# LANL-Bioinformatics/PCRamp

Measured on AMD Instinct MI355X. Metric: primer-pair x target amplification evals/sec, higher is better.
Workload: dtype u32

## Files before the change

### pcramp_amd/csrc/pcr_device.hip

```cpp
#include <hip/hip_runtime.h>
#include <cstring>
#include <rocprim/device/device_radix_sort.hpp>

#include <stdint.h>
#include <string.h>
#include <math.h>
#include <stdlib.h>
#include <string>
#include <vector>
#include <chrono>
#include <algorithm>
#include <unordered_map>
#include <type_traits>
#include <thread>
#include <mutex>
#include <condition_variable>
#include <functional>
#include <memory>

#include "../../include/pcramp_hip.h"
#include "pcr_host.hpp"

using pcrhost::Planes;

// ... 528 lines not shown
	uint32_t bucket_cap = 64;
	DevBuf<uint32_t> irr_perm; uint32_t irr_size_count[256];
	DevBuf<uint4> planes;
	DevBuf<uint32_t> valid, nib, tb, blk_seq, tile_seq, tile_pos0, irr_off, degen_tiles;
	uint32_t *valid_d() const { return valid.p + S2_VALID_FRONT; }
	uint32_t *tb_d() const { return tb.p + S2_TB_FRONT; }
	DevBuf<uint8_t> tile_degen; uint32_t n_degen_tiles = 0;
	DevBuf<TileDesc> tile_desc;
	DevBuf<uint64_t> d_len, d_blk_off, d_nblk_real;
	DevBuf<uint8_t> d_active;
	std::vector<uint8_t> has_eos; DevBuf<uint8_t> d_has_eos;
	DevBuf<IrrDev> irr;
	DevBuf<IrrScan> irr_scan;
	DevBuf<uint32_t> irx_first, irx_last, irx_words, irx_sums; bool irx_valid = false, irx_usable = false;
	uint32_t irr_n_multi = 0;
	DevBuf<uint32_t> pix_first, pix_last, pix_sums, blk_info, blk_local, blk_tile0; DevBuf<uint4> pix_ent; std::vector<uint32_t> pix_count_h; uint64_t pix_generation = 0; bool pix_valid = false, pix_usable = false;
	DevBuf<uint8_t> codes; DevBuf<uint64_t> d_code_off; bool have_codes = false;
	bool have_db = false;
	uint32_t n_entries = 0;
	uint32_t db_cap = 0;
	uint64_t n_slots = 0;
	DevBuf<DevEntry> db;
	DevBuf<uint32_t> touched;
	DevBuf<uint32_t> ctrl;
	uint32_t n_touched = 0;
	bool touched_built = false;
	uint32_t *d_seg_hi = nullptr;
	void release()
	{
		d_weight.release(); tile_desc.release(); irr_scan.release(); irx_first.release(); irx_last.release(); irx_words.release(); irx_sums.release(); pix_first.release(); pix_last.release(); pix_ent.release(); pix_sums.release(); blk_info.release(); blk_local.release(); blk_tile0.release(); irr_perm.release(); planes.release(); valid.release(); nib.release(); tb.release(); degen_tiles.release(); tile_degen.release(); blk_seq.release(); tile_seq.release(); tile_pos0.release();
		irr_off.release(); d_len.release(); d_blk_off.release();
		d_nblk_real.release(); d_active.release(); d_has_eos.release(); irr.release(); db.release(); touched.release(); ctrl.release(); codes.release(); d_code_off.release();
	}
};

}

struct HostPool {
	std::vector<std::thread> th;
	std::mutex m; std::condition_variable cv_go, cv_done;
	std::function<void(unsigned)> fn; unsigned n_parts = 0, next = 0, pending = 0; uint64_t gen = 0; bool stop = false;
	explicit HostPool(unsigned n_workers){ for(unsigned i = 0;i < n_workers;++i) th.emplace_back([this]{ work(); }); }
	~HostPool(){ { std::lock_guard<std::mutex> lk(m); stop = true; } cv_go.notify_all(); for(std::thread &t : th) t.join(); }
	unsigned size() const { return (unsigned)th.size(); }
	void work()
// ... 35 lines not shown
	pcrhost::PackFilter filt;
	SeqSet sets[PCR_N_SETS];
	DevBuf<uint32_t> best, counters, mask, status;
	int scan_version = 3;
	bool force_seed1 = false;
	std::vector<uint32_t> s2_seeds; std::vector<uint4> s2_masks; std::vector<uint8_t> s2_floors;
	std::vector<uint32_t> s2_group_end, s2_group_offmask, s2_group_or, s2_group_nor;
	struct S2Key { uint32_t a, c, g, t, floor_; bool operator==(const S2Key &o) const { return a == o.a && c == o.c && g == o.g && t == o.t && floor_ == o.floor_; } };
	struct S2KeyHash { size_t operator()(const S2Key &k) const { uint64_t h = 0x9E3779B97F4A7C15ull; for(uint32_t v : {k.a, k.c, k.g, k.t, k.floor_}){ h ^= v; h *= 0x100000001B3ull; h ^= h >> 29; } return (size_t)h; } };
	struct S2Entry { std::vector<uint32_t> seeds;  uint32_t off_mask; bool seedable; uint4 mask;
		std::vector<uint32_t> chunks; uint32_t chunks_total = 0; uint64_t chunks_gen = 0;  };
	std::unordered_map<S2Key, S2Entry, S2KeyHash> s2_cache;
	std::vector<pcrhost::Seed> s2_tmp;
	struct S3Launch { Seed3Slices W; uint32_t n_chunks, per_wg, slice_cap, n_irr_wg; };
	std::vector<S3Launch> s3_launch;
	std::vector<uint32_t> s3_prefix; bool no_seed3 = false, s3_attr_set = false;
	bool s2_attr_set = false; uint32_t s2_dbg = 0; bool no_irr_index = false;
	std::vector<uint32_t> s1_seeds; std::unordered_map<S2Key, S2Entry, S2KeyHash> s1_cache;
	DevBuf<uint32_t> s1_image, s1_heads, s1_multi, s1_part;
	bool host_seed_tables = false;
	DevBuf<Hit> hits;
	DevBuf<uint64_t> bits_fr, bits_rf;
	DevBuf<OligoDev> oligos;
	DevBuf<SwJob> sw_jobs; DevBuf<SwOut> sw_out; DevBuf<uint8_t> sw_q, sw_qlen, sw_t, entry_codes, entry_lens;
	DevBuf<AmpRec> amp_recs, amp_recs2; DevBuf<BgPairDev> bg_pairs;
	DevBuf<uint64_t> amp_keys; DevBuf<uint32_t> amp_pkeys, amp_pair_start; DevBuf<uint8_t> sort_tmp;
	DevBuf<thermo::Job> th_jobs; DevBuf<thermo::JobOut> th_out; DevBuf<int> th_dg; DevBuf<uint2> th_map; DevBuf<uint32_t> th_bad;
	float th_dg_salt = -1.0f;
	DevBuf<unsigned long long> th_dbg; bool th_attr_set = false;
	std::vector<thermo::Job> th_host_jobs; std::vector<thermo::JobOut> th_host_res;
	uint8_t *sw_pin = nullptr, *sw_pin_dev = nullptr; hipEvent_t sw_done[2] = {nullptr, nullptr};
// ... 193 lines not shown
	hipLaunchKernelGGL(k_scan_blocks, dim3(n_blocks), dim3(1024), 0, ctx->stream, S.irx_last.p, S.irx_first.p, IRX_KEYS, S.irx_sums.p);
	hipLaunchKernelGGL(k_scan_sums, dim3(1), dim3(1024), 0, ctx->stream, S.irx_sums.p, n_blocks);
	hipLaunchKernelGGL(k_scan_add, dim3(n_blocks), dim3(1024), 0, ctx->stream, S.irx_first.p, S.irx_last.p, IRX_KEYS, S.irx_sums.p);
	HIP_TRY(hipGetLastError());
	if(S.n_irr){
		hipLaunchKernelGGL(k_irx_scatter, dim3((S.n_irr + 255)/256), dim3(256), 0, ctx->stream, S.irr.p, S.n_irr, S.irx_last.p, S.irx_words.p);
		HIP_TRY(hipGetLastError());
	}
	S.irx_valid = true;
	return PCR_OK;
}

int ensure_pos_index(pcr_ctx *ctx, SeqSet &S)
{
	if(S.pix_valid) return PCR_OK;
	S.pix_valid = true; S.pix_usable = false;
	if(S.total_blocks == 0 || S.total_blocks*32 >= (uint64_t(1) << 32) - 64) return PCR_OK;
	int rc;
	if((rc = S.pix_first.ensure(PIX_CODES + 4)) != PCR_OK) return rc;
	if((rc = S.pix_last.ensure(PIX_CODES + 4)) != PCR_OK) return rc;
	const uint32_t n_blocks = (PIX_CODES + 4095u)/4096u;
	if((rc = S.pix_sums.ensure(n_blocks + 4)) != PCR_OK) return rc;
	if((rc = S.pix_ent.ensure(S.total_blocks*32 + 64)) != PCR_OK) return rc;
	{
		if(S.n >= (1u << 30)){ return PCR_OK; }
		if((rc = S.blk_info.ensure(S.total_blocks + 1)) != PCR_OK) return rc;
		if((rc = S.blk_local.ensure(S.total_blocks + 1)) != PCR_OK) return rc;
		std::vector<uint32_t> tile0((size_t)S.n + 1);
		uint64_t t0 = 0;
		for(uint32_t q = 0;q < S.n;++q){ tile0[q] = (uint32_t)t0; t0 += (S.len[q] >= 32) ? (S.len[q] - 7 + TILE_POS - 1)/TILE_POS : 0; }
		tile0[S.n] = (uint32_t)t0;
		if(t0 >= (uint64_t(1) << 32)) return PCR_OK;
		if((rc = S.blk_tile0.ensure((size_t)S.n + 1)) != PCR_OK) return rc;
		HIP_TRY(hipMemcpyAsync(S.blk_tile0.p, tile0.data(), ((size_t)S.n + 1)*sizeof(uint32_t), hipMemcpyHostToDevice, ctx->stream));
		hipLaunchKernelGGL(k_blk_info, dim3((unsigned)((S.total_blocks + 255)/256)), dim3(256), 0, ctx->stream, S.blk_seq.p, S.d_blk_off.p, S.d_len.p,
			S.blk_tile0.p, S.tile_degen.p, S.d_active.p, S.total_blocks, S.blk_info.p, S.blk_local.p);
		HIP_TRY(hipGetLastError());
		HIP_TRY(hipStreamSynchronize(ctx->stream));
	}
	HIP_TRY(hipMemsetAsync(S.pix_last.p, 0, (size_t)PIX_CODES*sizeof(uint32_t), ctx->stream));
	const unsigned grid = (unsigned)((S.total_blocks + 255)/256);
	hipLaunchKernelGGL(k_pix_build<false>, dim3(grid), dim3(256), 0, ctx->stream, S.tb_d(), S.blk_seq.p, S.d_blk_off.p, S.d_len.p, S.total_blocks, S.pix_last.p, (uint4 *)nullptr);
	hipLaunchKernelGGL(k_scan_blocks, dim3(n_blocks), dim3(1024), 0, ctx->stream, S.pix_last.p, S.pix_first.p, PIX_CODES, S.pix_sums.p);
	hipLaunchKernelGGL(k_scan_sums, dim3(1), dim3(1024), 0, ctx->stream, S.pix_sums.p, n_blocks);
	hipLaunchKernelGGL(k_scan_add, dim3(n_blocks), dim3(1024), 0, ctx->stream, S.pix_first.p, S.pix_last.p, PIX_CODES, S.pix_sums.p);
	hipLaunchKernelGGL(k_pix_build<true>, dim3(grid), dim3(256), 0, ctx->stream, S.tb_d(), S.blk_seq.p, S.d_blk_off.p, S.d_len.p, S.total_blocks, S.pix_last.p, S.pix_ent.p);
	HIP_TRY(hipGetLastError());
	{
		std::vector<uint32_t> first(PIX_CODES), last(PIX_CODES);
		HIP_TRY(hipMemcpyAsync(first.data(), S.pix_first.p, (size_t)PIX_CODES*sizeof(uint32_t), hipMemcpyDeviceToHost, ctx->stream));
		HIP_TRY(hipMemcpyAsync(last.data(), S.pix_last.p, (size_t)PIX_CODES*sizeof(uint32_t), hipMemcpyDeviceToHost, ctx->stream));
		HIP_TRY(hipStreamSynchronize(ctx->stream));
		S.pix_count_h.resize(PIX_CODES);
		for(uint32_t c = 0;c < PIX_CODES;++c) S.pix_count_h[c] = last[c] - first[c];
		static uint64_t generations = 0;
		S.pix_generation = ++generations;
	}
	S.pix_usable = true;
	return PCR_OK;
}

int run_valid(pcr_ctx *ctx, SeqSet &S, uint64_t first_block, uint64_t n_blocks)
{
	if(n_blocks == 0) return PCR_OK;
	const unsigned threads = 256;
	const unsigned grid = (unsigned)((n_blocks + threads - 1)/threads);
	hipLaunchKernelGGL(k_valid, dim3(grid), dim3(threads), 0, ctx->stream, S.planes.p, S.d_blk_off.p, S.blk_seq.p,
		S.d_nblk_real.p, S.valid_d(), S.total_blocks, ctx->filt.max_degen, ctx->filt.gc_ok, first_block, n_blocks);
	HIP_TRY(hipGetLastError());
	return PCR_OK;
}

int build_tile_desc(pcr_ctx *ctx, SeqSet &S)
// ... 822 lines not shown
		const uint32_t *P = ctx->s3_prefix.data() + g_prefix;
		g_prefix += (size_t)ns + 1;
		pcr_ctx::S3Launch &L = ctx->s3_launch[g];
		L.n_irr_wg = with_irr ? std::min<uint32_t>((ns + 16u*(uint32_t)(wg_threads/64) - 1u)/(16u*(uint32_t)(wg_threads/64)), G_all/4u) : 0u;
		const uint32_t G = G_all - L.n_irr_wg;
		L.n_chunks = P[ns]; L.per_wg = std::max<uint32_t>(1u, (L.n_chunks + G - 1u)/G); L.slice_cap = 2;
		if(ns == 0) continue;
		uint32_t at = 0;
		for(uint32_t w = 0;w <= G;++w){
			const uint64_t target = (uint64_t)w*L.per_wg;
			while(at + 1u < ns && P[at + 1u] <= target) ++at;
			L.W.start[w] = at;
		}
		for(uint32_t w = G + 1;w <= S3_MAX_WG;++w) L.W.start[w] = at;
		for(uint32_t w = 0;w < G;++w) L.slice_cap = std::max(L.slice_cap, std::min(L.W.start[w + 1] + 2u, ns + 1u) - L.W.start[w]);
		if(17*(size_t)ctx->s2_group_nor[g] + 8*(size_t)L.slice_cap + 64 > S3_LDS_BUDGET) return false;
	}
	return true;
}

void plan_seed1(pcr_ctx *ctx, const std::vector<pcrhost::Candidate> &cand, std::vector<uint32_t> &or_seed, std::vector<uint32_t> &or_plain, uint32_t &irr_off_mask)
{
	const uint32_t n_or = 2*(uint32_t)cand.size();
	std::vector<uint32_t> &out = ctx->s1_seeds;
	out.clear();
	irr_off_mask = 0;
	if(ctx->s1_cache.size() > 16384) ctx->s1_cache.clear();
	std::vector<const pcr_ctx::S2Entry *> ent(n_or);
	size_t total = 0;
	for(uint32_t o = 0;o < n_or;++o){
		const pcrhost::Candidate &c = cand[o >> 1];
// ... 239 lines not shown
		&& ctx->s3_prefix.size() == ctx->s2_seeds.size() + ctx->s2_group_end.size();
	bool dev_tables = false;
	if(!use_seed2 && ctx->scan_version == 3 && !ctx->host_seed_tables && !optimize_5 && !optimize_3 && n_or <= S1_MAX_OR){
		plan_seed1(ctx, cand, or_seed, or_plain, irr_off_mask);
		dev_tables = true;
	}
	if(use_seed2 || dev_tables){  }
	else if(ctx->scan_version == 3 && n_or <= 65535){
		const int prc = plan_seed_host(ctx, cand, H, or_seed, or_plain, irr_off_mask);
		if(ctx->seed_count.size() == 65536){ for(const pcrhost::Seed &sd : H.seeds){ ctx->seed_count[sd.code] = 0; ctx->seed_own[sd.code] = 0; } }
		if(prc != PCR_OK) return prc;
	}
	else{ for(uint32_t o = 0;o < n_or;++o) or_plain.push_back(o); }
	SeedTables ST; memset(&ST, 0, sizeof(ST));
	Seed2Tables ST2; memset(&ST2, 0, sizeof(ST2));
	const uint32_t *d_s3_prefix = nullptr;
	const size_t n_seeds = use_seed2 ? ctx->s2_seeds.size() : dev_tables ? ctx->s1_seeds.size() : H.seeds.size() + H.n_inherited;
	if(ctx->debug_log) fprintf(stderr, "[pcramp] scan plan: %u candidates, %zu seeded orientations (%zu seeds), %zu plain, %u/%u IUPAC tiles, %u-slot buckets\n",
		ncand, or_seed.size(), n_seeds, or_plain.size(), S.n_degen_tiles, S.n_tiles, S.bucket_cap);
	Scan2Tables tab_plain, tab_seedset;
	const bool need_plain = (ctx->scan_version != 1) && !or_plain.empty();
	const bool need_seedset = !or_seed.empty() && S.n_degen_tiles > 0;
	if(need_plain) build_scan2_tables(cand, or_plain, tab_plain);
	if(need_seedset) build_scan2_tables(cand, or_seed, tab_seedset);
	const uint32_t *d_tab_plain = nullptr, *d_bias_plain = nullptr, *d_map_plain = nullptr;
	const uint32_t *d_tab_seedset = nullptr, *d_bias_seedset = nullptr, *d_map_seedset = nullptr;
	{
		size_t bytes = ncand*(2*sizeof(uint4) + sizeof(uint32_t)) + 1024;
		bytes += (tab_plain.tab.size() + tab_plain.bias.size() + or_plain.size() + 256)*sizeof(uint32_t);
		bytes += (tab_seedset.tab.size() + tab_seedset.bias.size() + or_seed.size() + 256)*sizeof(uint32_t);
		bytes += (H.image.size() + H.heads.size() + H.multi.size() + 64)*sizeof(uint32_t);
		std::vector<uint4> &masks2 = ctx->s2_masks; std::vector<uint8_t> &floors2 = ctx->s2_floors;
		if(use_seed2){
			floors2.assign(((size_t)n_or + 15) & ~size_t(15), 0);
			for(uint32_t o = 0;o < n_or;++o) floors2[o] = (uint8_t)std::min<uint32_t>(cand[o >> 1].floor_, 255u);
			bytes += masks2.size()*sizeof(uint4) + floors2.size() + ctx->s2_seeds.size()*sizeof(uint32_t) + 512;
			if(use_seed3) bytes += ctx->s3_prefix.size()*sizeof(uint32_t) + 64;
		}
		const bool build_tables = dev_tables && !or_seed.empty();
		if(build_tables) bytes += ctx->s1_seeds.size()*sizeof(uint32_t) + 256;
		std::vector<OligoDev> ol;
		size_t bits_bytes = 0;
		bool fuse = false;
		if(fa && fa->n_pairs){
			bits_bytes = (size_t)fa->n_pairs*((S.n + 63)/64)*sizeof(uint64_t);
			fuse = ((uintptr_t)fa->d_fr % 16 == 0) && ((uintptr_t)fa->d_rf % 16 == 0) && (bits_bytes % 16 == 0);
			if(fuse){ build_oligos(fa->pairs, fa->n_pairs, fa->a, ol); bytes += ol.size()*sizeof(OligoDev) + 64; }
		}
		timer.next(1);
		{
			const uint64_t gen = S.ctrl.generation;
			if((rc = S.ctrl.ensure(8 + 2*(size_t)S.n + 4)) != PCR_OK) return rc;
// ... 26 lines not shown
			ST.multi = H.multi.empty() ? ST.heads : st.put(H.multi.data(), H.multi.size());
		}
		const uint32_t *d_s1_seeds = nullptr;
		if(build_tables){
			d_s1_seeds = st.put(ctx->s1_seeds.data(), ctx->s1_seeds.size());
			if((rc = ctx->s1_image.ensure(SEED_IMAGE_WORDS)) != PCR_OK) return rc;
			if((rc = ctx->s1_heads.ensure(2*(size_t)S1_MAX_SEEDS)) != PCR_OK) return rc;
			if((rc = ctx->s1_multi.ensure(S1_MAX_SEEDS)) != PCR_OK) return rc;
			ST.image = ctx->s1_image.p; ST.heads = ctx->s1_heads.p; ST.multi = ctx->s1_multi.p; ST.flat = 1;
		}
		if(use_seed2){
			ST2.seeds = st.put(ctx->s2_seeds.data(), ctx->s2_seeds.size());
			ST2.masks = st.put(masks2.data(), masks2.size());
			ST2.floors = st.put(floors2.data(), floors2.size());
			ST2.n_seeds = (uint32_t)ctx->s2_seeds.size(); ST2.n_or = n_or;
			if(use_seed3) d_s3_prefix = st.put(ctx->s3_prefix.data(), ctx->s3_prefix.size());
		}
		if(fuse){
			fa->d_oligos = st.put(ol.data(), ol.size());
			fa->staged = true;
			if(lean) st.seal(ctx->mail_seq + 1);
			else if((rc = st.ship(S.ctrl.p, (8 + 2*(size_t)S.n)*sizeof(uint32_t), fa->d_fr, bits_bytes, fa->d_rf, bits_bytes, ctx->mail_seq + 1)) != PCR_OK) return rc;
		}
		else if((rc = st.ship(S.ctrl.p, (8 + 2*(size_t)S.n)*sizeof(uint32_t), nullptr, 0, nullptr, 0, ctx->mail_seq + 1)) != PCR_OK) return rc;
		if(build_tables){
			if((rc = ctx->s1_part.ensure(2*S1_GROUPS)) != PCR_OK) return rc;
			hipLaunchKernelGGL(k_seed_tables<false>, dim3(S1_GROUPS), dim3(S1_BUILD_THREADS), 0, ctx->stream, d_s1_seeds, (uint32_t)ctx->s1_seeds.size(),
				ctx->s1_part.p, ctx->s1_image.p, ctx->s1_heads.p, ctx->s1_multi.p);
			hipLaunchKernelGGL(k_seed_tables<true>, dim3(S1_GROUPS), dim3(S1_BUILD_THREADS), 0, ctx->stream, d_s1_seeds, (uint32_t)ctx->s1_seeds.size(),
				ctx->s1_part.p, ctx->s1_image.p, ctx->s1_heads.p, ctx->s1_multi.p);
			HIP_TRY(hipGetLastError());
// ... 57 lines not shown
						Tg.masks = ST2.masks + (size_t)or0; Tg.floors = ST2.floors + or0; Tg.n_or = g_or; Tg.or_base = or0;
						g_begin = ctx->s2_group_end[g];
						if(Tg.n_seeds == 0){ g_prefix += 1u; continue; }
						const size_t dyn = (size_t)g_or*sizeof(uint4) + (((size_t)g_or + 15) & ~size_t(15)) + 8*((size_t)Tg.n_seeds + 64) + 16;
						IrrArgs2 IA; IA.scan = S.irr_scan.p; IA.irr = S.irr.p; IA.n_live = n_live;
						IA.off_mask = ctx->s2_group_offmask[g];
						IA.exhaustive = first_launch ? 1u : 0u;
						IA.ix_first = IA.ix_last = IA.ix_words = nullptr; IA.min_cws = std::min<uint32_t>(min_oligo_length, 255u);
						if(!or_plain.empty()){
							IA.off_mask = 0;
							if(!first_launch) IA.n_live = 0;
						}
						else if(irr_by_index){
							IA.ix_first = S.irx_first.p; IA.ix_last = S.irx_last.p; IA.ix_words = S.irx_words.p; IA.n_live = 0;
						}
						if(ctx->debug_log) fprintf(stderr, "[pcramp] k_seed2: %u workgroups, %u seeds of orientations %u..%u (group %zu of %zu), %zu + %zu B of LDS\n", sgrid.x, Tg.n_seeds,
							or0, or0 + g_or - 1, g + 1, ctx->s2_group_end.size(), sizeof(S2Shared), dyn);
						S2Clear Z = { nullptr, 0u, nullptr, 0u, nullptr };
						if(lean && !cleared_bits){
							Z.z0 = (uint4 *)fa->d_fr; Z.z1 = (uint4 *)fa->d_rf; Z.n0 = Z.n1 = (uint32_t)(lean_bits_bytes/16); Z.ctrl = d_counters;
							cleared_bits = true;
						}
						if(use_seed3){
							Seed3Tables T3; T3.seeds = Tg.seeds; T3.chunk_prefix = d_s3_prefix + g_prefix; T3.masks = Tg.masks; T3.floors = Tg.floors;
							g_prefix += Tg.n_seeds + 1u;
							T3.n_seeds = Tg.n_seeds; T3.n_or = Tg.n_or; T3.or_base = Tg.or_base;
							T3.pix_first = S.pix_first.p; T3.pix_last = S.pix_last.p; T3.pix_ent = S.pix_ent.p;
							Seed3Set Q3 = { S.valid_d(), S.blk_info.p, S.blk_local.p, S.d_active.p };
							int s3_wg = 0;
							const uint32_t G = seed3_grid(ctx, &s3_wg);
							const pcr_ctx::S3Launch &L3 = ctx->s3_launch[g];
							T3.n_chunks = L3.n_chunks; T3.per_wg = L3.per_wg; T3.slice_cap = L3.slice_cap;
							T3.n_irr_wg = IA.ix_first ? L3.n_irr_wg : 0u;
							const Seed3Slices &W3 = L3.W;
							const size_t dyn3 = (size_t)g_or*sizeof(uint4) + 2*(size_t)T3.slice_cap*sizeof(uint32_t) + (((size_t)g_or + 15) & ~size_t(15)) + 16;
							if(!ctx->s3_attr_set){
								HIP_TRY(hipFuncSetAttribute((const void *)k_seed3<512>, hipFuncAttributeMaxDynamicSharedMemorySize, 128*1024));
								HIP_TRY(hipFuncSetAttribute((const void *)k_seed3<1024>, hipFuncAttributeMaxDynamicSharedMemorySize, 128*1024));
								ctx->s3_attr_set = true;
							}
							if(s3_wg == 1024) hipLaunchKernelGGL(k_seed3<1024>, dim3(G), dim3(1024), dyn3, ctx->stream, T3, Q3, IA, ctx->d_cand_fwd, ctx->d_cand_floor, sink, Z, W3);
							else hipLaunchKernelGGL(k_seed3<512>, dim3(G), dim3(512), dyn3, ctx->stream, T3, Q3, IA, ctx->d_cand_fwd, ctx->d_cand_floor, sink, Z, W3);
						}
						else if(ctx->s2_dbg)
							hipLaunchKernelGGL(k_seed2<true>, sgrid, sblock, dyn, ctx->stream, S.tb_d(), S.valid_d(), S.tile_desc.p, S.n_tiles, Tg, S.d_active.p, ctx->d_cand_fwd, ctx->d_cand_floor, ncand, IA, sink,
							ctx->s2_dbg, Z);
						else
							hipLaunchKernelGGL(k_seed2<false>, sgrid, sblock, dyn, ctx->stream, S.tb_d(), S.valid_d(), S.tile_desc.p, S.n_tiles, Tg, S.d_active.p, ctx->d_cand_fwd, ctx->d_cand_floor, ncand, IA, sink,
							ctx->s2_dbg, Z);
						HIP_TRY(hipGetLastError());
// ... 467 lines not shown
```

### pcramp_amd/csrc/pcr_scan_seed3.inc

```

constexpr uint32_t PIX_CODES = 1u << 18;
constexpr uint32_t S3_BATCH = 8;

template<bool SCATTER>
__global__ void k_pix_build(const uint32_t *__restrict__ tb, const uint32_t *__restrict__ blk_seq, const uint64_t *__restrict__ blk_off,
	const uint64_t *__restrict__ len, uint64_t total_blocks, uint32_t *__restrict__ count_or_cursor, uint4 *__restrict__ ent)
{
	const uint64_t b = (uint64_t)blockIdx.x*blockDim.x + threadIdx.x;
	if(b >= total_blocks) return;
	const uint32_t seq = blk_seq[b];
	const int64_t p0 = (int64_t)(b - blk_off[seq])*32, L = (int64_t)len[seq];
	uint32_t w[8];
#pragma unroll
	for(int k = 0;k < 8;++k) w[k] = tb[(int64_t)2*(int64_t)b - 2 + k];
#pragma unroll
	for(int i = 0;i < 32;++i){
		if(p0 + i + 9 > L) break;
		const uint32_t code = ((i < 16) ? funnel(w[2], w[3], 2*i) : funnel(w[3], w[4], 2*(i - 16))) & S2_CODE_MASK;
		if(SCATTER){
			const uint32_t at = atomicAdd(&count_or_cursor[code], 1u);
			const int jl = (i + 9) >> 4, sl = 2*((i + 9) & 15);
			const int jr = (i + 41) >> 4, sr = 2*((i + 41) & 15);
			const uint32_t l_lo = funnel(w[jl], w[jl + 1], sl), l_hi = funnel(w[jl + 1], w[jl + 2], sl) & 0x3FFFu;
			const uint32_t r_lo = funnel(w[jr], w[jr + 1], sr), r_hi = funnel(w[jr + 1], w[jr + 2], sr) & 0x3FFFu;
			ent[at] = make_uint4((uint32_t)(b*32 + (uint64_t)i), l_lo, l_hi | (r_lo << 14), (r_lo >> 18) | (r_hi << 14));
		}
		else atomicAdd(&count_or_cursor[code], 1u);
	}
}

struct Seed3Tables {
	const uint32_t *seeds;
	const uint32_t *chunk_prefix;
	const uint4 *masks; const uint8_t *floors;
	uint32_t n_seeds, n_or, or_base;
	const uint32_t *pix_first, *pix_last; const uint4 *pix_ent;
	uint32_t n_chunks, per_wg, slice_cap;
	uint32_t n_irr_wg;
};
constexpr uint32_t S3_MAX_WG = 512;
constexpr uint32_t S3_MAX_OR = 448, S3_MAX_SEEDS = 1u << 16;
struct Seed3Slices { uint32_t start[S3_MAX_WG + 1]; };
struct Seed3Set {
	const uint32_t *valid, *blk_info, *blk_local; const uint8_t *active;
};
constexpr uint32_t BLK_SEQ_MASK = 0x3FFFFFFFu, BLK_INACTIVE = 0x40000000u, BLK_DEGEN = 0x80000000u;

__global__ void k_blk_info(const uint32_t *__restrict__ blk_seq, const uint64_t *__restrict__ blk_off, const uint64_t *__restrict__ len,
	const uint32_t *__restrict__ tile0, const uint8_t *__restrict__ tile_degen, const uint8_t *__restrict__ active, uint64_t total_blocks,
	uint32_t *__restrict__ blk_info, uint32_t *__restrict__ blk_local)
{
	const uint64_t b = (uint64_t)blockIdx.x*blockDim.x + threadIdx.x;
	if(b >= total_blocks) return;
	const uint32_t q = blk_seq[b];
	const uint64_t bl = b - blk_off[q], tile = bl >> 5;
	const uint32_t nt = tile0[q + 1] - tile0[q];
	const bool degen = tile < nt && tile_degen[tile0[q] + tile];
// ... 36 lines not shown
			if(((e.meta >> 8) & 0xFFu) < IA.min_cws || !Q.active[e.seq]) continue;
			const uint32_t n = match_count(e.w.a, e.w.c, e.w.g, e.w.t, cand_fwd[c]);
			if(n >= cand_floor[c]) record_hit(sink, e.seq, c, make_key(e.seq, e.loc, e.meta & 0xFF, 1, (e.meta >> 16) & 0xFF), n);
		}
	}
}

template<uint32_t S3_THREADS>
__global__ __launch_bounds__(S3_THREADS) __attribute__((amdgpu_waves_per_eu(8, 8))) void k_seed3(Seed3Tables T3, Seed3Set Q, IrrArgs2 IA, const uint4 *__restrict__ cand_fwd, const uint32_t *__restrict__ cand_floor,
	HitSink sink, S2Clear Z, Seed3Slices W)
{
	extern __shared__ uint4 s3_dyn[];
	uint4 *const masks = s3_dyn;
	uint32_t *const prefix = (uint32_t *)(masks + T3.n_or);
	uint32_t *const seeds = prefix + T3.slice_cap;
	uint8_t *const floors = (uint8_t *)(seeds + T3.slice_cap);
	const uint32_t wave = threadIdx.x >> 6, lane = threadIdx.x & 63u;
	for(uint32_t i = blockIdx.x*S3_THREADS + threadIdx.x;i < Z.n0;i += gridDim.x*S3_THREADS) Z.z0[i] = make_uint4(0, 0, 0, 0);
	for(uint32_t i = blockIdx.x*S3_THREADS + threadIdx.x;i < Z.n1;i += gridDim.x*S3_THREADS) Z.z1[i] = make_uint4(0, 0, 0, 0);
	if(Z.ctrl && blockIdx.x == 0 && threadIdx.x == 0){ Z.ctrl[1] = 0; Z.ctrl[3] = 0; }
	for(uint32_t i = threadIdx.x;i < T3.n_or;i += S3_THREADS){ masks[i] = T3.masks[i]; floors[i] = T3.floors[i]; }
	constexpr uint32_t S3_WAVES = S3_THREADS/64;
	if(blockIdx.x < T3.n_irr_wg){
		if(IA.ix_first) s3_irregular(T3, Q, IA, cand_fwd, cand_floor, sink, blockIdx.x*S3_WAVES + wave, T3.n_irr_wg*S3_WAVES, lane);
		return;
	}
	const uint32_t wg = blockIdx.x - T3.n_irr_wg, n_wg = gridDim.x - T3.n_irr_wg;
	const uint32_t s_lo = W.start[wg];
	const uint32_t n_slice = min(min(W.start[wg + 1] + 2u, T3.n_seeds + 1u) - s_lo, T3.slice_cap);
	for(uint32_t i = threadIdx.x;i < n_slice;i += S3_THREADS){ prefix[i] = T3.chunk_prefix[s_lo + i]; seeds[i] = (s_lo + i < T3.n_seeds) ? T3.seeds[s_lo + i] : 0u; }
	__syncthreads();
	const uint32_t gw = wg*S3_WAVES + wave, n_gw = n_wg*S3_WAVES;
	const uint32_t q_lo = wg*T3.per_wg, q_hi = min(q_lo + T3.per_wg, T3.n_chunks);
	for(uint32_t q0 = q_lo + wave;q0 < q_hi;q0 += S3_WAVES*S3_BATCH){
		uint32_t c_first = 0, c_cnt = 0, c_sd = 0;
		{
			const uint32_t q = q0 + lane*S3_WAVES;
			if(lane < S3_BATCH && q < q_hi){
				uint32_t lo = 0, hi = n_slice - 1u;
				while(hi - lo > 1u){ const uint32_t mid = (lo + hi) >> 1; if(prefix[mid] <= q) lo = mid; else hi = mid; }
				c_sd = seeds[lo];
				const uint32_t code = c_sd >> 14;
				const uint32_t f = T3.pix_first[code], e = T3.pix_last[code], j0 = (q - prefix[lo])*64u;
				c_first = f + j0; c_cnt = (e - f) - j0;
			}
		}
		uint4 en[S3_BATCH];
#pragma unroll
		for(int b = 0;b < (int)S3_BATCH;++b){
			const uint32_t first = s2_rl(c_first, b), cnt = s2_rl(c_cnt, b);
			en[b] = make_uint4(0xFFFFFFFFu, 0, 0, 0);
			if(lane < cnt) en[b] = T3.pix_ent[first + lane];
		}
		uint32_t cnt_b[S3_BATCH], g[S3_BATCH]; bool pass_b[S3_BATCH];
#pragma unroll
		for(int b = 0;b < (int)S3_BATCH;++b){
			const uint32_t sdv = s2_rl(c_sd, b);
			const uint32_t off = (sdv >> 9) & 31u, local = sdv & 0x1FFu, code = sdv >> 14;
			g[b] = en[b].x;
			const uint32_t r_lo = funnel(en[b].z, en[b].w, 14);
			const uint4 cx = make_uint4(en[b].y << 2, (funnel(en[b].y, en[b].z, 30) & 0xFFFFu) | (code << 16), (code >> 16) | (r_lo << 2), en[b].w >> 12);
			const uint32_t in = 24u - off, sh = 2u*(in & 15u);
			const uint32_t a0 = (in < 16u) ? funnel(cx.x, cx.y, sh) : funnel(cx.y, cx.z, sh);
			const uint32_t a1 = (in < 16u) ? funnel(cx.y, cx.z, sh) : funnel(cx.z, cx.w, sh);
			cnt_b[b] = (uint32_t)__popc(s2_mux(a0, a1, masks[local]));
			pass_b[b] = g[b] != 0xFFFFFFFFu && cnt_b[b] >= floors[local] && g[b] >= off;
		}
		uint32_t vw[S3_BATCH], info[S3_BATCH], bl[S3_BATCH];
#pragma unroll
		for(int b = 0;b < (int)S3_BATCH;++b){
			vw[b] = 0; info[b] = 0; bl[b] = 0;
			if(pass_b[b]){
				const uint32_t ws = g[b] - ((s2_rl(c_sd, b) >> 9) & 31u);
				vw[b] = Q.valid[ws >> 5]; info[b] = Q.blk_info[ws >> 5]; bl[b] = Q.blk_local[ws >> 5];
			}
		}
#pragma unroll
		for(int b = 0;b < (int)S3_BATCH;++b){
			if(!pass_b[b]) continue;
			const uint32_t sdv = s2_rl(c_sd, b);
			const uint32_t ws = g[b] - ((sdv >> 9) & 31u), seq = info[b] & BLK_SEQ_MASK;
// ... 10 lines not shown
```

Baseline: 19.30 billion.

## Split position index entries into separate planes loaded only when needed

Replaces the 16-byte interleaved position-index entry with four separate u32 arrays: position, left context, right context and far context. The seed3 kernel works out from each seed's offset and its mask's occupied span which context words the mask actually uses, and loads only those, which is meant to cut gather bandwidth. A separate fill kernel now builds the context arrays, per-orientation floors become 32-bit words that carry the span, and index allocation checks free memory and falls back cleanly. Memory use rises when all planes are kept, and LDS per orientation grows.

```diff
diff --git a/pcramp_amd/csrc/pcr_device.hip b/pcramp_amd/csrc/pcr_device.hip
--- a/pcramp_amd/csrc/pcr_device.hip
+++ b/pcramp_amd/csrc/pcr_device.hip
@@ -566,7 +566,7 @@
 	DevBuf<IrrScan> irr_scan;
 	DevBuf<uint32_t> irx_first, irx_last, irx_words, irx_sums; bool irx_valid = false, irx_usable = false;
 	uint32_t irr_n_multi = 0;
-	DevBuf<uint32_t> pix_first, pix_last, pix_sums, blk_info, blk_local, blk_tile0; DevBuf<uint4> pix_ent; std::vector<uint32_t> pix_count_h; uint64_t pix_generation = 0; bool pix_valid = false, pix_usable = false;
+	DevBuf<uint32_t> pix_first, pix_last, pix_sums, blk_info, blk_local, blk_tile0, pix_pos, pix_l, pix_r, pix_far; std::vector<uint32_t> pix_count_h; uint64_t pix_generation = 0; bool pix_valid = false, pix_usable = false;
 	DevBuf<uint8_t> codes; DevBuf<uint64_t> d_code_off; bool have_codes = false;
 	bool have_db = false;
 	uint32_t n_entries = 0;
@@ -580,7 +580,7 @@
 	uint32_t *d_seg_hi = nullptr;
 	void release()
 	{
-		d_weight.release(); tile_desc.release(); irr_scan.release(); irx_first.release(); irx_last.release(); irx_words.release(); irx_sums.release(); pix_first.release(); pix_last.release(); pix_ent.release(); pix_sums.release(); blk_info.release(); blk_local.release(); blk_tile0.release(); irr_perm.release(); planes.release(); valid.release(); nib.release(); tb.release(); degen_tiles.release(); tile_degen.release(); blk_seq.release(); tile_seq.release(); tile_pos0.release();
+		d_weight.release(); tile_desc.release(); irr_scan.release(); irx_first.release(); irx_last.release(); irx_words.release(); irx_sums.release(); pix_first.release(); pix_last.release(); pix_pos.release(); pix_l.release(); pix_r.release(); pix_far.release(); pix_sums.release(); blk_info.release(); blk_local.release(); blk_tile0.release(); irr_perm.release(); planes.release(); valid.release(); nib.release(); tb.release(); degen_tiles.release(); tile_degen.release(); blk_seq.release(); tile_seq.release(); tile_pos0.release();
 		irr_off.release(); d_len.release(); d_blk_off.release();
 		d_nblk_real.release(); d_active.release(); d_has_eos.release(); irr.release(); db.release(); touched.release(); ctrl.release(); codes.release(); d_code_off.release();
 	}
@@ -646,7 +646,7 @@
 	std::vector<pcrhost::Seed> s2_tmp;
 	struct S3Launch { Seed3Slices W; uint32_t n_chunks, per_wg, slice_cap, n_irr_wg; };
 	std::vector<S3Launch> s3_launch;
-	std::vector<uint32_t> s3_prefix; bool no_seed3 = false, s3_attr_set = false;
+	std::vector<uint32_t> s3_prefix, s3_floors; bool no_seed3 = false, s3_attr_set = false;
 	bool s2_attr_set = false; uint32_t s2_dbg = 0; bool no_irr_index = false;
 	std::vector<uint32_t> s1_seeds; std::unordered_map<S2Key, S2Entry, S2KeyHash> s1_cache;
 	DevBuf<uint32_t> s1_image, s1_heads, s1_multi, s1_part;
@@ -870,24 +870,39 @@
 int ensure_pos_index(pcr_ctx *ctx, SeqSet &S)
 {
 	if(S.pix_valid) return PCR_OK;
-	S.pix_valid = true; S.pix_usable = false;
-	if(S.total_blocks == 0 || S.total_blocks*32 >= (uint64_t(1) << 32) - 64) return PCR_OK;
-	int rc;
-	if((rc = S.pix_first.ensure(PIX_CODES + 4)) != PCR_OK) return rc;
-	if((rc = S.pix_last.ensure(PIX_CODES + 4)) != PCR_OK) return rc;
+	S.pix_usable = false;
+	auto decline = [&](const char *why){
+		S.pix_first.release(); S.pix_last.release(); S.pix_sums.release(); S.pix_pos.release(); S.pix_l.release(); S.pix_r.release(); S.pix_far.release();
+		S.blk_info.release(); S.blk_local.release(); S.blk_tile0.release();
+		(void)hipGetLastError();
+		if(ctx->debug_log) fprintf(stderr, "[pcramp] position index declined: %s\n", why);
+		S.pix_usable = false; S.pix_valid = true;
+		return PCR_OK;
+	};
+	if(S.total_blocks == 0 || S.total_blocks*32 >= (uint64_t(1) << 32) - 64) return decline("positions are 32-bit");
+	if(S.n >= (1u << 30)) return decline("too many sequences");
+	std::vector<uint32_t> tile0((size_t)S.n + 1);
+	uint64_t t0 = 0;
+	for(uint32_t q = 0;q < S.n;++q){ tile0[q] = (uint32_t)t0; t0 += (S.len[q] >= 32) ? (S.len[q] - 7 + TILE_POS - 1)/TILE_POS : 0; }
+	tile0[S.n] = (uint32_t)t0;
+	if(t0 >= (uint64_t(1) << 32)) return decline("too many tiles");
+	const size_t n_ent = (size_t)S.total_blocks*32 + 64;
 	const uint32_t n_blocks = (PIX_CODES + 4095u)/4096u;
-	if((rc = S.pix_sums.ensure(n_blocks + 4)) != PCR_OK) return rc;
-	if((rc = S.pix_ent.ensure(S.total_blocks*32 + 64)) != PCR_OK) return rc;
+	const uint64_t need = (uint64_t)n_ent*16 + (uint64_t)(S.total_blocks + 1)*8 + ((uint64_t)S.n + 1)*4 + (uint64_t)(2*(PIX_CODES + 4) + n_blocks + 4)*4;
+	if(const char *v = getenv("PCRAMP_PIX_MAX_BYTES")){
+		if(need > strtoull(v, nullptr, 0)) return decline("larger than PCRAMP_PIX_MAX_BYTES");
+	}
+	else{
+		size_t free_b = 0, total_b = 0;
+		if(hipMemGetInfo(&free_b, &total_b) != hipSuccess) return decline("hipMemGetInfo failed");
+		const uint64_t held = (uint64_t)(S.pix_pos.cap + S.pix_l.cap + S.pix_r.cap + S.pix_far.cap + S.blk_info.cap + S.blk_local.cap)*4;
+		if(need > held && need - held + need/4 + (uint64_t(1) << 30) > free_b) return decline("not enough free device memory");
+	}
+	if(S.pix_first.ensure(PIX_CODES + 4) != PCR_OK || S.pix_last.ensure(PIX_CODES + 4) != PCR_OK || S.pix_sums.ensure(n_blocks + 4) != PCR_OK
+		|| S.pix_pos.ensure(n_ent) != PCR_OK || S.pix_l.ensure(n_ent) != PCR_OK || S.pix_r.ensure(n_ent) != PCR_OK || S.pix_far.ensure(n_ent) != PCR_OK
+		|| S.blk_info.ensure(S.total_blocks + 1) != PCR_OK || S.blk_local.ensure(S.total_blocks + 1) != PCR_OK || S.blk_tile0.ensure((size_t)S.n + 1) != PCR_OK)
+		return decline("allocation failed");
 	{
-		if(S.n >= (1u << 30)){ return PCR_OK; }
-		if((rc = S.blk_info.ensure(S.total_blocks + 1)) != PCR_OK) return rc;
-		if((rc = S.blk_local.ensure(S.total_blocks + 1)) != PCR_OK) return rc;
-		std::vector<uint32_t> tile0((size_t)S.n + 1);
-		uint64_t t0 = 0;
-		for(uint32_t q = 0;q < S.n;++q){ tile0[q] = (uint32_t)t0; t0 += (S.len[q] >= 32) ? (S.len[q] - 7 + TILE_POS - 1)/TILE_POS : 0; }
-		tile0[S.n] = (uint32_t)t0;
-		if(t0 >= (uint64_t(1) << 32)) return PCR_OK;
-		if((rc = S.blk_tile0.ensure((size_t)S.n + 1)) != PCR_OK) return rc;
 		HIP_TRY(hipMemcpyAsync(S.blk_tile0.p, tile0.data(), ((size_t)S.n + 1)*sizeof(uint32_t), hipMemcpyHostToDevice, ctx->stream));
 		hipLaunchKernelGGL(k_blk_info, dim3((unsigned)((S.total_blocks + 255)/256)), dim3(256), 0, ctx->stream, S.blk_seq.p, S.d_blk_off.p, S.d_len.p,
 			S.blk_tile0.p, S.tile_degen.p, S.d_active.p, S.total_blocks, S.blk_info.p, S.blk_local.p);
@@ -896,11 +911,12 @@
 	}
 	HIP_TRY(hipMemsetAsync(S.pix_last.p, 0, (size_t)PIX_CODES*sizeof(uint32_t), ctx->stream));
 	const unsigned grid = (unsigned)((S.total_blocks + 255)/256);
-	hipLaunchKernelGGL(k_pix_build<false>, dim3(grid), dim3(256), 0, ctx->stream, S.tb_d(), S.blk_seq.p, S.d_blk_off.p, S.d_len.p, S.total_blocks, S.pix_last.p, (uint4 *)nullptr);
+	hipLaunchKernelGGL(k_pix_build<false>, dim3(grid), dim3(256), 0, ctx->stream, S.tb_d(), S.blk_seq.p, S.d_blk_off.p, S.d_len.p, S.total_blocks, S.pix_last.p, (uint32_t *)nullptr);
 	hipLaunchKernelGGL(k_scan_blocks, dim3(n_blocks), dim3(1024), 0, ctx->stream, S.pix_last.p, S.pix_first.p, PIX_CODES, S.pix_sums.p);
 	hipLaunchKernelGGL(k_scan_sums, dim3(1), dim3(1024), 0, ctx->stream, S.pix_sums.p, n_blocks);
 	hipLaunchKernelGGL(k_scan_add, dim3(n_blocks), dim3(1024), 0, ctx->stream, S.pix_first.p, S.pix_last.p, PIX_CODES, S.pix_sums.p);
-	hipLaunchKernelGGL(k_pix_build<true>, dim3(grid), dim3(256), 0, ctx->stream, S.tb_d(), S.blk_seq.p, S.d_blk_off.p, S.d_len.p, S.total_blocks, S.pix_last.p, S.pix_ent.p);
+	hipLaunchKernelGGL(k_pix_build<true>, dim3(grid), dim3(256), 0, ctx->stream, S.tb_d(), S.blk_seq.p, S.d_blk_off.p, S.d_len.p, S.total_blocks, S.pix_last.p, S.pix_pos.p);
+	hipLaunchKernelGGL(k_pix_fill, dim3((unsigned)((S.total_blocks*32 + 255)/256)), dim3(256), 0, ctx->stream, S.tb_d(), S.pix_last.p, S.pix_pos.p, S.pix_l.p, S.pix_r.p, S.pix_far.p);
 	HIP_TRY(hipGetLastError());
 	{
 		std::vector<uint32_t> first(PIX_CODES), last(PIX_CODES);
@@ -912,7 +928,7 @@
 		static uint64_t generations = 0;
 		S.pix_generation = ++generations;
 	}
-	S.pix_usable = true;
+	S.pix_usable = true; S.pix_valid = true;
 	return PCR_OK;
 }
 
@@ -1765,7 +1781,7 @@
 		}
 		for(uint32_t w = G + 1;w <= S3_MAX_WG;++w) L.W.start[w] = at;
 		for(uint32_t w = 0;w < G;++w) L.slice_cap = std::max(L.slice_cap, std::min(L.W.start[w + 1] + 2u, ns + 1u) - L.W.start[w]);
-		if(17*(size_t)ctx->s2_group_nor[g] + 8*(size_t)L.slice_cap + 64 > S3_LDS_BUDGET) return false;
+		if(20*(size_t)ctx->s2_group_nor[g] + 8*(size_t)L.slice_cap + 64 > S3_LDS_BUDGET) return false;
 	}
 	return true;
 }
@@ -2035,7 +2051,7 @@
 	else{ for(uint32_t o = 0;o < n_or;++o) or_plain.push_back(o); }
 	SeedTables ST; memset(&ST, 0, sizeof(ST));
 	Seed2Tables ST2; memset(&ST2, 0, sizeof(ST2));
-	const uint32_t *d_s3_prefix = nullptr;
+	const uint32_t *d_s3_prefix = nullptr, *d_s3_floors = nullptr;
 	const size_t n_seeds = use_seed2 ? ctx->s2_seeds.size() : dev_tables ? ctx->s1_seeds.size() : H.seeds.size() + H.n_inherited;
 	if(ctx->debug_log) fprintf(stderr, "[pcramp] scan plan: %u candidates, %zu seeded orientations (%zu seeds), %zu plain, %u/%u IUPAC tiles, %u-slot buckets\n",
 		ncand, or_seed.size(), n_seeds, or_plain.size(), S.n_degen_tiles, S.n_tiles, S.bucket_cap);
@@ -2056,7 +2072,14 @@
 			floors2.assign(((size_t)n_or + 15) & ~size_t(15), 0);
 			for(uint32_t o = 0;o < n_or;++o) floors2[o] = (uint8_t)std::min<uint32_t>(cand[o >> 1].floor_, 255u);
 			bytes += masks2.size()*sizeof(uint4) + floors2.size() + ctx->s2_seeds.size()*sizeof(uint32_t) + 512;
-			if(use_seed3) bytes += ctx->s3_prefix.size()*sizeof(uint32_t) + 64;
+			if(use_seed3){
+				ctx->s3_floors.resize(n_or);
+				for(uint32_t o = 0;o < n_or;++o){
+					const Planes &m = (o & 1u) ? cand[o >> 1].rc : cand[o >> 1].fwd;
+					ctx->s3_floors[o] = s3_floor_word(cand[o >> 1].floor_, m.a | m.c | m.g | m.t);
+				}
+				bytes += ctx->s3_prefix.size()*sizeof(uint32_t) + ctx->s3_floors.size()*sizeof(uint32_t) + 128;
+			}
 		}
 		const bool build_tables = dev_tables && !or_seed.empty();
 		if(build_tables) bytes += ctx->s1_seeds.size()*sizeof(uint32_t) + 256;
@@ -2113,7 +2136,7 @@
 			ST2.masks = st.put(masks2.data(), masks2.size());
 			ST2.floors = st.put(floors2.data(), floors2.size());
 			ST2.n_seeds = (uint32_t)ctx->s2_seeds.size(); ST2.n_or = n_or;
-			if(use_seed3) d_s3_prefix = st.put(ctx->s3_prefix.data(), ctx->s3_prefix.size());
+			if(use_seed3){ d_s3_prefix = st.put(ctx->s3_prefix.data(), ctx->s3_prefix.size()); d_s3_floors = st.put(ctx->s3_floors.data(), ctx->s3_floors.size()); }
 		}
 		if(fuse){
 			fa->d_oligos = st.put(ol.data(), ol.size());
@@ -2201,7 +2224,7 @@
 						else if(irr_by_index){
 							IA.ix_first = S.irx_first.p; IA.ix_last = S.irx_last.p; IA.ix_words = S.irx_words.p; IA.n_live = 0;
 						}
-						if(ctx->debug_log) fprintf(stderr, "[pcramp] k_seed2: %u workgroups, %u seeds of orientations %u..%u (group %zu of %zu), %zu + %zu B of LDS\n", sgrid.x, Tg.n_seeds,
+						if(ctx->debug_log && !use_seed3) fprintf(stderr, "[pcramp] k_seed2: %u workgroups, %u seeds of orientations %u..%u (group %zu of %zu), %zu + %zu B of LDS\n", sgrid.x, Tg.n_seeds,
 							or0, or0 + g_or - 1, g + 1, ctx->s2_group_end.size(), sizeof(S2Shared), dyn);
 						S2Clear Z = { nullptr, 0u, nullptr, 0u, nullptr };
 						if(lean && !cleared_bits){
@@ -2209,10 +2232,10 @@
 							cleared_bits = true;
 						}
 						if(use_seed3){
-							Seed3Tables T3; T3.seeds = Tg.seeds; T3.chunk_prefix = d_s3_prefix + g_prefix; T3.masks = Tg.masks; T3.floors = Tg.floors;
+							Seed3Tables T3; T3.seeds = Tg.seeds; T3.chunk_prefix = d_s3_prefix + g_prefix; T3.masks = Tg.masks; T3.floors = d_s3_floors + or0;
 							g_prefix += Tg.n_seeds + 1u;
 							T3.n_seeds = Tg.n_seeds; T3.n_or = Tg.n_or; T3.or_base = Tg.or_base;
-							T3.pix_first = S.pix_first.p; T3.pix_last = S.pix_last.p; T3.pix_ent = S.pix_ent.p;
+							T3.pix_first = S.pix_first.p; T3.pix_last = S.pix_last.p; T3.pix_pos = S.pix_pos.p; T3.pix_l = S.pix_l.p; T3.pix_r = S.pix_r.p; T3.pix_far = S.pix_far.p;
 							Seed3Set Q3 = { S.valid_d(), S.blk_info.p, S.blk_local.p, S.d_active.p };
 							int s3_wg = 0;
 							const uint32_t G = seed3_grid(ctx, &s3_wg);
@@ -2220,7 +2243,18 @@
 							T3.n_chunks = L3.n_chunks; T3.per_wg = L3.per_wg; T3.slice_cap = L3.slice_cap;
 							T3.n_irr_wg = IA.ix_first ? L3.n_irr_wg : 0u;
 							const Seed3Slices &W3 = L3.W;
-							const size_t dyn3 = (size_t)g_or*sizeof(uint4) + 2*(size_t)T3.slice_cap*sizeof(uint32_t) + (((size_t)g_or + 15) & ~size_t(15)) + 16;
+							const size_t dyn3 = (size_t)g_or*sizeof(uint4) + 2*(size_t)T3.slice_cap*sizeof(uint32_t) + (size_t)g_or*sizeof(uint32_t) + 16;
+							if(ctx->debug_log){
+								uint64_t planned = 0; uint32_t n_l = 0, n_r = 0, n_far = 0;
+								const uint32_t *sd = ctx->s2_seeds.data() + (g_begin - Tg.n_seeds);
+								for(uint32_t k = 0;k < Tg.n_seeds;++k){
+									const uint32_t need = s3_need((sd[k] >> 9) & 31u, ctx->s3_floors[or0 + (sd[k] & 0x1FFu)]);
+									planned += (uint64_t)S.pix_count_h[sd[k] >> 14]*4u*(1u + (need & 1u) + ((need >> 1) & 1u) + ((need >> 2) & 1u));
+									n_l += need & 1u; n_r += (need >> 1) & 1u; n_far += (need >> 2) & 1u;
+								}
+								fprintf(stderr, "[pcramp] k_seed3: %u workgroups (%u for the irregular words), %u seeds of orientations %u..%u (group %zu of %zu), %u chunks, %llu planned bytes (seeds reading left %u, right %u, far %u), %zu B of LDS\n",
+									G, T3.n_irr_wg, T3.n_seeds, or0, or0 + g_or - 1, g + 1, ctx->s2_group_end.size(), T3.n_chunks, (unsigned long long)planned, n_l, n_r, n_far, dyn3);
+							}
 							if(!ctx->s3_attr_set){
 								HIP_TRY(hipFuncSetAttribute((const void *)k_seed3<512>, hipFuncAttributeMaxDynamicSharedMemorySize, 128*1024));
 								HIP_TRY(hipFuncSetAttribute((const void *)k_seed3<1024>, hipFuncAttributeMaxDynamicSharedMemorySize, 128*1024));
diff --git a/pcramp_amd/csrc/pcr_scan_seed3.inc b/pcramp_amd/csrc/pcr_scan_seed3.inc
--- a/pcramp_amd/csrc/pcr_scan_seed3.inc
+++ b/pcramp_amd/csrc/pcr_scan_seed3.inc
@@ -4,43 +4,64 @@
 
 template<bool SCATTER>
 __global__ void k_pix_build(const uint32_t *__restrict__ tb, const uint32_t *__restrict__ blk_seq, const uint64_t *__restrict__ blk_off,
-	const uint64_t *__restrict__ len, uint64_t total_blocks, uint32_t *__restrict__ count_or_cursor, uint4 *__restrict__ ent)
+	const uint64_t *__restrict__ len, uint64_t total_blocks, uint32_t *__restrict__ count_or_cursor, uint32_t *__restrict__ pos)
 {
 	const uint64_t b = (uint64_t)blockIdx.x*blockDim.x + threadIdx.x;
 	if(b >= total_blocks) return;
 	const uint32_t seq = blk_seq[b];
 	const int64_t p0 = (int64_t)(b - blk_off[seq])*32, L = (int64_t)len[seq];
-	uint32_t w[8];
-#pragma unroll
-	for(int k = 0;k < 8;++k) w[k] = tb[(int64_t)2*(int64_t)b - 2 + k];
+	uint32_t w[3];
+#pragma unroll
+	for(int k = 0;k < 3;++k) w[k] = tb[(int64_t)2*(int64_t)b + k];
 #pragma unroll
 	for(int i = 0;i < 32;++i){
 		if(p0 + i + 9 > L) break;
-		const uint32_t code = ((i < 16) ? funnel(w[2], w[3], 2*i) : funnel(w[3], w[4], 2*(i - 16))) & S2_CODE_MASK;
-		if(SCATTER){
-			const uint32_t at = atomicAdd(&count_or_cursor[code], 1u);
-			const int jl = (i + 9) >> 4, sl = 2*((i + 9) & 15);
-			const int jr = (i + 41) >> 4, sr = 2*((i + 41) & 15);
-			const uint32_t l_lo = funnel(w[jl], w[jl + 1], sl), l_hi = funnel(w[jl + 1], w[jl + 2], sl) & 0x3FFFu;
-			const uint32_t r_lo = funnel(w[jr], w[jr + 1], sr), r_hi = funnel(w[jr + 1], w[jr + 2], sr) & 0x3FFFu;
-			ent[at] = make_uint4((uint32_t)(b*32 + (uint64_t)i), l_lo, l_hi | (r_lo << 14), (r_lo >> 18) | (r_hi << 14));
-		}
-		else atomicAdd(&count_or_cursor[code], 1u);
-	}
+		const uint32_t code = ((i < 16) ? funnel(w[0], w[1], 2*i) : funnel(w[1], w[2], 2*(i - 16))) & S2_CODE_MASK;
+		const uint32_t at = atomicAdd(&count_or_cursor[code], 1u);
+		if(SCATTER) pos[at] = (uint32_t)(b*32 + (uint64_t)i);
+	}
+}
+
+__device__ __forceinline__ uint32_t pix_bases16(const uint32_t *__restrict__ tb, int64_t base)
+{
+	const int64_t j = base >> 4;
+	return funnel(tb[j], tb[j + 1], 2u*(uint32_t)(base & 15));
+}
+__global__ void k_pix_fill(const uint32_t *__restrict__ tb, const uint32_t *__restrict__ run_end, const uint32_t *__restrict__ pos,
+	uint32_t *__restrict__ l, uint32_t *__restrict__ r, uint32_t *__restrict__ far)
+{
+	const uint64_t e = (uint64_t)blockIdx.x*blockDim.x + threadIdx.x;
+	if(e >= run_end[PIX_CODES - 1]) return;
+	const int64_t p = (int64_t)pos[e];
+	l[e] = pix_bases16(tb, p - 16);
+	r[e] = pix_bases16(tb, p + 9);
+	far[e] = (pix_bases16(tb, p - 23) & 0x3FFFu) | ((pix_bases16(tb, p + 25) & 0x3FFFu) << 16);
 }
 
 struct Seed3Tables {
 	const uint32_t *seeds;
 	const uint32_t *chunk_prefix;
-	const uint4 *masks; const uint8_t *floors;
+	const uint4 *masks; const uint32_t *floors;
 	uint32_t n_seeds, n_or, or_base;
-	const uint32_t *pix_first, *pix_last; const uint4 *pix_ent;
+	const uint32_t *pix_first, *pix_last;
+	const uint32_t *pix_pos, *pix_l, *pix_r, *pix_far;
 	uint32_t n_chunks, per_wg, slice_cap;
 	uint32_t n_irr_wg;
 };
 constexpr uint32_t S3_MAX_WG = 512;
 constexpr uint32_t S3_MAX_OR = 448, S3_MAX_SEEDS = 1u << 16;
 struct Seed3Slices { uint32_t start[S3_MAX_WG + 1]; };
+constexpr uint32_t S3_NEED_L = 1u, S3_NEED_R = 2u, S3_NEED_FAR = 4u;
+__host__ __device__ inline uint32_t s3_floor_word(uint32_t floor, uint32_t occupied)
+{
+	const uint32_t s0 = occupied ? (uint32_t)__builtin_ctz(occupied) : 0u, s1 = occupied ? 32u - (uint32_t)__builtin_clz(occupied) : 0u;
+	return (floor < 255u ? floor : 255u) | (s0 << 8) | (s1 << 16);
+}
+__host__ __device__ inline uint32_t s3_need(uint32_t off, uint32_t floor_word)
+{
+	const uint32_t s0 = (floor_word >> 8) & 0xFFu, s1 = (floor_word >> 16) & 0xFFu;
+	return (off > s0 ? S3_NEED_L : 0u) | (s1 > off + 9u ? S3_NEED_R : 0u) | ((off > s0 + 16u || s1 > off + 25u) ? S3_NEED_FAR : 0u);
+}
 struct Seed3Set {
 	const uint32_t *valid, *blk_info, *blk_local; const uint8_t *active;
 };
@@ -107,7 +128,7 @@
 	uint4 *const masks = s3_dyn;
 	uint32_t *const prefix = (uint32_t *)(masks + T3.n_or);
 	uint32_t *const seeds = prefix + T3.slice_cap;
-	uint8_t *const floors = (uint8_t *)(seeds + T3.slice_cap);
+	uint32_t *const floors = seeds + T3.slice_cap;
 	const uint32_t wave = threadIdx.x >> 6, lane = threadIdx.x & 63u;
 	for(uint32_t i = blockIdx.x*S3_THREADS + threadIdx.x;i < Z.n0;i += gridDim.x*S3_THREADS) Z.z0[i] = make_uint4(0, 0, 0, 0);
 	for(uint32_t i = blockIdx.x*S3_THREADS + threadIdx.x;i < Z.n1;i += gridDim.x*S3_THREADS) Z.z1[i] = make_uint4(0, 0, 0, 0);
@@ -126,7 +147,7 @@
 	const uint32_t gw = wg*S3_WAVES + wave, n_gw = n_wg*S3_WAVES;
 	const uint32_t q_lo = wg*T3.per_wg, q_hi = min(q_lo + T3.per_wg, T3.n_chunks);
 	for(uint32_t q0 = q_lo + wave;q0 < q_hi;q0 += S3_WAVES*S3_BATCH){
-		uint32_t c_first = 0, c_cnt = 0, c_sd = 0;
+		uint32_t c_first = 0, c_cnt = 0, c_sd = 0, c_need = 0;
 		{
 			const uint32_t q = q0 + lane*S3_WAVES;
 			if(lane < S3_BATCH && q < q_hi){
@@ -136,28 +157,32 @@
 				const uint32_t code = c_sd >> 14;
 				const uint32_t f = T3.pix_first[code], e = T3.pix_last[code], j0 = (q - prefix[lo])*64u;
 				c_first = f + j0; c_cnt = (e - f) - j0;
+				c_need = s3_need((c_sd >> 9) & 31u, floors[c_sd & 0x1FFu]);
 			}
 		}
-		uint4 en[S3_BATCH];
-#pragma unroll
-		for(int b = 0;b < (int)S3_BATCH;++b){
-			const uint32_t first = s2_rl(c_first, b), cnt = s2_rl(c_cnt, b);
-			en[b] = make_uint4(0xFFFFFFFFu, 0, 0, 0);
-			if(lane < cnt) en[b] = T3.pix_ent[first + lane];
-		}
-		uint32_t cnt_b[S3_BATCH], g[S3_BATCH]; bool pass_b[S3_BATCH];
+		uint32_t g[S3_BATCH], e_l[S3_BATCH], e_r[S3_BATCH], e_far[S3_BATCH];
+#pragma unroll
+		for(int b = 0;b < (int)S3_BATCH;++b){
+			const uint32_t first = s2_rl(c_first, b), cnt = s2_rl(c_cnt, b), need = s2_rl(c_need, b);
+			g[b] = 0; e_l[b] = 0; e_r[b] = 0; e_far[b] = 0;
+			if(lane < cnt){
+				g[b] = T3.pix_pos[first + lane];
+				if(need & S3_NEED_L) e_l[b] = T3.pix_l[first + lane];
+				if(need & S3_NEED_R) e_r[b] = T3.pix_r[first + lane];
+				if(need & S3_NEED_FAR) e_far[b] = T3.pix_far[first + lane];
+			}
+		}
+		uint32_t cnt_b[S3_BATCH]; bool pass_b[S3_BATCH];
 #pragma unroll
 		for(int b = 0;b < (int)S3_BATCH;++b){
 			const uint32_t sdv = s2_rl(c_sd, b);
 			const uint32_t off = (sdv >> 9) & 31u, local = sdv & 0x1FFu, code = sdv >> 14;
-			g[b] = en[b].x;
-			const uint32_t r_lo = funnel(en[b].z, en[b].w, 14);
-			const uint4 cx = make_uint4(en[b].y << 2, (funnel(en[b].y, en[b].z, 30) & 0xFFFFu) | (code << 16), (code >> 16) | (r_lo << 2), en[b].w >> 12);
+			const uint4 cx = make_uint4(((e_far[b] & 0x3FFFu) << 2) | (e_l[b] << 16), (e_l[b] >> 16) | (code << 16), (code >> 16) | (e_r[b] << 2), (e_r[b] >> 30) | ((e_far[b] >> 14) & 0xFFFCu));
 			const uint32_t in = 24u - off, sh = 2u*(in & 15u);
 			const uint32_t a0 = (in < 16u) ? funnel(cx.x, cx.y, sh) : funnel(cx.y, cx.z, sh);
 			const uint32_t a1 = (in < 16u) ? funnel(cx.y, cx.z, sh) : funnel(cx.z, cx.w, sh);
 			cnt_b[b] = (uint32_t)__popc(s2_mux(a0, a1, masks[local]));
-			pass_b[b] = g[b] != 0xFFFFFFFFu && cnt_b[b] >= floors[local] && g[b] >= off;
+			pass_b[b] = lane < s2_rl(c_cnt, b) && cnt_b[b] >= (floors[local] & 0xFFu) && g[b] >= off;
 		}
 		uint32_t vw[S3_BATCH], info[S3_BATCH], bl[S3_BATCH];
 #pragma unroll
```

Result: slower. 14.35 billion (-25.6%).
